# mathaiml5/NBody-simulation-parallel

Measured on AMD Instinct MI355X. Metric: body-pair interactions/sec at N=2^20 (all-pairs force + kick/drift step), higher is better.
Workload: dtype f32

## Files before the change

### include/nbody_hip.h

```cpp
#ifndef NBODY_HIP_H
#define NBODY_HIP_H

#include <stddef.h>
#include <stdint.h>

#ifdef __cplusplus
extern "C" {
#endif
#if defined(__GNUC__)
#pragma GCC visibility push(default)
#endif

#define NBX_ABI_VERSION 5

enum {
    NBX_OK = 0,
    NBX_ERR_INVALID = 1,
    NBX_ERR_NO_DEVICE = 2,
    NBX_ERR_HIP = 3,
    NBX_ERR_ALLOC = 4,
    NBX_ERR_STATE = 5
};

#define NBX_REFERENCE_G 4.471e-21
// ... 123 lines not shown
int nbx_ctx_get_accel(nbx_ctx* ctx, float* accel_out);
int nbx_ctx_download_bodies(nbx_ctx* ctx, void* bodies, size_t body_stride_bytes);

int nbx_ctx_energy(nbx_ctx* ctx, double G, double* kinetic, double* potential);

int nbx_ctx_synchronize(nbx_ctx* ctx);

int nbx_ctx_set_tuning(nbx_ctx* ctx, int source_splits, int variant);
enum { NBX_CLOSE_CANDIDATE_PAIRS = 0, NBX_CLOSE_SORTED_CELLS = 1, NBX_CLOSE_GUARDED_KERNEL = 2, NBX_CLOSE_NONE = 3 };
int nbx_ctx_close_set_mode(nbx_ctx* ctx, int* mode, unsigned* candidates_seen, unsigned* bad_seen);

int nbx_ctx_set_softening(nbx_ctx* ctx, double epsilon);
enum { NBX_FORCE_LAW_REFERENCE = 0, NBX_FORCE_LAW_NEWTON = 1 };
int nbx_ctx_set_law(nbx_ctx* ctx, int law);
int nbx_ctx_set_refine(nbx_ctx* ctx, double rel_tolerance, double sigma_factor);
int nbx_ctx_refine_stats(nbx_ctx* ctx, unsigned* selected, unsigned* refined);
int nbx_ctx_get_aux(nbx_ctx* ctx, double* out);
int nbx_ctx_effective_tuning(nbx_ctx* ctx, int* variant, int* source_splits);
int nbx_num_variants(void);
const char* nbx_variant_name(int variant);
int nbx_default_variant(void);

int nbx_ctx_kernel_time(nbx_ctx* ctx, float* mean_ms, int* launches);
int nbx_ctx_refine_time(nbx_ctx* ctx, float* total_ms);

int nbx_variant_kernel_symbol(int variant, int dim, int mixed_mode, char* buf, size_t len);
int nbx_ctx_enable_clock_stamps(nbx_ctx* ctx, int on);
int nbx_ctx_shader_clock(nbx_ctx* ctx, double* median_mhz, double* min_mhz, double* max_mhz, int* workgroups);
int nbx_measure_valu_ceiling(int device, double target_ms, double* tflops, double* shader_mhz);

// ... 31 lines not shown
```

### nbody-simulation-parallel_amd/capi.py

```python
from __future__ import annotations

import ctypes
import os
from typing import Optional, Tuple

import numpy as np

NBX_OK = 0
NBX_ERR_INVALID, NBX_ERR_NO_DEVICE, NBX_ERR_HIP, NBX_ERR_ALLOC, NBX_ERR_STATE = 1, 2, 3, 4, 5
SRC_ALL, SRC_LOCAL, SRC_REMOTE = 0, 1, 2
REFERENCE_G = 4.471e-21

_PKG_DIR = os.path.dirname(os.path.abspath(__file__))
LIB_PATH = os.environ.get("NBODY_HIP_LIBRARY") or os.path.join(_PKG_DIR, "libnbody_hip.so")

_c = ctypes
_vp, _sz, _i, _d = _c.c_void_p, _c.c_size_t, _c.c_int, _c.c_double
_pf, _pd, _pi = _c.POINTER(_c.c_float), _c.POINTER(_c.c_double), _c.POINTER(_c.c_int)
ABI = [
    ("nbx_abi_version", _i, []),
    ("nbx_strerror", _c.c_char_p, [_i]),
    ("nbx_last_error_detail", _c.c_char_p, []),
    ("nbx_device_count", _i, [_pi]),
    ("nbx_warmup", _i, [_i]),
# ... 49 lines not shown
    ("nbx_ctx_compute_accel", _i, [_vp, _i]),
    ("nbx_ctx_kick_drift", _i, [_vp, _d, _d]),
    ("nbx_ctx_kick_drift2", _i, [_vp, _d, _d, _d]),
    ("nbx_ctx_step_kdk", _i, [_vp, _d, _d, _i]),
    ("nbx_ctx_step", _i, [_vp, _d, _d, _i]),
    ("nbx_ctx_get_forces", _i, [_vp, _d, _vp]),
    ("nbx_ctx_accuracy", _i, [_vp, _d, _vp, _pd]),
    ("nbx_ctx_get_accel", _i, [_vp, _vp]),
    ("nbx_ctx_download_bodies", _i, [_vp, _vp, _sz]),
    ("nbx_ctx_energy", _i, [_vp, _d, _pd, _pd]),
    ("nbx_ctx_synchronize", _i, [_vp]),
    ("nbx_ctx_set_tuning", _i, [_vp, _i, _i]),
    ("nbx_ctx_set_softening", _i, [_vp, _d]),
    ("nbx_ctx_set_law", _i, [_vp, _i]),
    ("nbx_ctx_set_refine", _i, [_vp, _d, _d]),
    ("nbx_ctx_refine_stats", _i, [_vp, _c.POINTER(_c.c_uint), _c.POINTER(_c.c_uint)]),
    ("nbx_ctx_get_aux", _i, [_vp, _vp]),
    ("nbx_ctx_close_set_mode", _i, [_vp, _pi, _c.POINTER(_c.c_uint), _c.POINTER(_c.c_uint)]),
    ("nbx_ctx_effective_tuning", _i, [_vp, _pi, _pi]),
    ("nbx_num_variants", _i, []),
    ("nbx_variant_name", _c.c_char_p, [_i]),
    ("nbx_default_variant", _i, []),
    ("nbx_ctx_kernel_time", _i, [_vp, _pf, _pi]),
    ("nbx_ctx_refine_time", _i, [_vp, _pf]),
    ("nbx_variant_kernel_symbol", _i, [_i, _i, _i, _c.c_char_p, _sz]),
    ("nbx_ctx_enable_clock_stamps", _i, [_vp, _i]),
    ("nbx_ctx_shader_clock", _i, [_vp, _pd, _pd, _pd, _pi]),
    ("nbx_measure_valu_ceiling", _i, [_i, _d, _pd, _pd]),
    ("nbx_node_create", _i, [_c.POINTER(_vp), _i, _pi, _i, _sz, _i]),
    ("nbx_node_destroy", _i, [_vp]),
# ... 438 lines not shown

    def set_softening(self, epsilon: float):
        self._ck(self.lib.nbx_ctx_set_softening(self.h, float(epsilon)), "nbx_ctx_set_softening")

    def close_set_mode(self) -> Tuple[str, int, int]:
        m, a, b = ctypes.c_int(0), ctypes.c_uint(0), ctypes.c_uint(0)
        self._ck(self.lib.nbx_ctx_close_set_mode(self.h, ctypes.byref(m), ctypes.byref(a), ctypes.byref(b)), "nbx_ctx_close_set_mode")
        return ("candidate_pairs", "sorted_cells", "guarded_kernel", "none")[m.value], a.value, b.value

    def set_law(self, law: int):
        self._ck(self.lib.nbx_ctx_set_law(self.h, int(law)), "nbx_ctx_set_law")

    def set_refine(self, rel_tolerance: float, sigma_factor: float = 0.0):
        self._ck(self.lib.nbx_ctx_set_refine(self.h, float(rel_tolerance), float(sigma_factor)), "nbx_ctx_set_refine")

    def refine_stats(self) -> Tuple[int, int]:
        a, b = ctypes.c_uint(0), ctypes.c_uint(0)
        self._ck(self.lib.nbx_ctx_refine_stats(self.h, ctypes.byref(a), ctypes.byref(b)), "nbx_ctx_refine_stats")
        return a.value, b.value

    def aux(self) -> np.ndarray:
        out = np.empty(self.count, dtype=np.float64)
        self._ck(self.lib.nbx_ctx_get_aux(self.h, out.ctypes.data), "nbx_ctx_get_aux")
        return out

    def effective_tuning(self) -> Tuple[str, int]:
        v, s = ctypes.c_int(0), ctypes.c_int(0)
        self._ck(self.lib.nbx_ctx_effective_tuning(self.h, ctypes.byref(v), ctypes.byref(s)), "nbx_ctx_effective_tuning")
        return self.lib.nbx_variant_name(v.value).decode(), s.value

# ... 185 lines not shown
```

### nbody-simulation-parallel_amd/csrc/force_kernel.hip

```cpp
#include "nbx_internal.h"

#include <climits>
#include <cmath>

namespace nbx {
namespace {


typedef float f2 __attribute__((ext_vector_type(2)));

template <int D>
__device__ __forceinline__ void interact(float sx, float sy, float sz, float sm,
                                         float ix, float iy, float iz,
                                         float& ax, float& ay, float& az) {
    const float dx = sx - ix;
    const float dy = sy - iy;
    float r2 = dx * dx;
    r2 = __builtin_fmaf(dy, dy, r2);
    float dz = 0.0f;
    if (D == 3) {
        dz = sz - iz;
        r2 = __builtin_fmaf(dz, dz, r2);
    }
    const float r2g = (r2 < kR2SkipF) ? __builtin_inff() : r2;
// ... 709 lines not shown
                for (int s = 1; s < a.splits; ++s) a.acc[((size_t)s * D + k) * a.pad + i] = 0.0f;
            }
        }
    }
}

template <int D>
__global__ __launch_bounds__(256) void refine_select_kernel(KArgs a) {
    const unsigned gid = blockIdx.x * 256u + threadIdx.x;
    const unsigned i = gid >> 2, part = gid & 3u;
    const bool in = i < a.count;
    double t = 0.0;
    if (in && part < (unsigned)D) {
#pragma unroll 8
        for (int s = 0; s < a.splits; ++s) t += (double)a.acc[((size_t)s * D + part) * a.pad + i];
        t = t * t;
    } else if (in && part == 3u) {
#pragma unroll 8
        for (int s = 0; s < a.grid_slices; ++s) t += (double)a.qsum[(size_t)s * a.pad + i];
    }
    const int base = (int)(threadIdx.x & 63u) & ~3;
    const double n2 = __shfl(t, base) + __shfl(t, base + 1) + (D == 3 ? __shfl(t, base + 2) : 0.0);
    const double Q = __shfl(t, base + 3);
    if (in && part == 0u) {
        const bool suspect = a.bad_flag[i] != 0u || !(Q * a.refine_c2 <= n2);
        if (suspect) {
            const unsigned slot = atomicAdd(&a.counters[3], 1u);
            if (slot < a.strict_cap) a.strict_list[slot] = i;
        }
    }
// ... 1 lines not shown

template <int D>
__global__ __launch_bounds__(256) void refine_fold_kernel(KArgs a) {
    const StrictLayout sl = strict_layout<D>(a);
    const unsigned lane = threadIdx.x & 63u;
    const unsigned long long items = (unsigned long long)sl.n * (unsigned)D;
    for (unsigned long long item = blockIdx.x * 4u + (threadIdx.x >> 6); item < items; item += gridDim.x * 4u) {
        const unsigned slot = (unsigned)(item / (unsigned)D), k = (unsigned)(item - (unsigned long long)slot * (unsigned)D);
        double v = 0.0;
        for (unsigned y = lane; y < sl.slices; y += 64u) v += a.strict_acc[((size_t)y * D + k) * sl.stride + slot];
        for (int off = 32; off > 0; off >>= 1) v += __shfl_xor(v, off);
        const unsigned i = a.strict_list[slot];
        const float hi = (float)v;
        if (lane == 0u) {
            a.acc[(size_t)k * a.pad + i] = hi;
            if (a.splits > 1) a.acc[((size_t)D + k) * a.pad + i] = (float)(v - (double)hi);
        }
        for (unsigned sp = 2u + lane; sp < (unsigned)a.splits; sp += 64u) a.acc[((size_t)sp * D + k) * a.pad + i] = 0.0f;
    }
}

template <int D, int SOFT>
__global__ __launch_bounds__(256, 8) void potential_kernel(KArgs a) {
    constexpr int TPL = 2;
    __shared__ float4 tile[2][kTile];
    const unsigned tid = threadIdx.x;
    unsigned bx, by;
    xcd_tile(bx, by);
    const unsigned tgt0 = bx * (256u * TPL) + tid;
    const float* __restrict__ tp = a.pos_all + (size_t)a.tgt_chunk * D * a.pad;
    float ix[TPL], iy[TPL], iz[TPL];
// ... 113 lines not shown
```

### nbody-simulation-parallel_amd/csrc/force_launch.hip

```cpp
#include "nbx_internal.h"
#include "sym_plan.h"

#include <cxxabi.h>

#include <climits>
#include <cstdio>
#include <cstdlib>
#include <cstring>
#include <vector>

namespace nbx {
namespace {

struct Table {
    std::vector<KernelVariant> v;
    int def = 0, def_exact = 0, def_two_rcp = 0;
    CloseKernels ck;
    Table() {
        int n = 0;
        const KernelVariant* a = kernel_variants(&n);
        for (int i = 0; i < n; ++i) v.push_back(a[i]);
        v.push_back(sym_kernel_variant());
        v.push_back(sym_dpp_kernel_variant());
        for (size_t i = 0; i < v.size(); ++i) {
// ... 74 lines not shown
    a.pad = L.pad;
    a.count = L.count;
    a.tiles_per_chunk = L.pad / kTile;
    a.total_tiles = (unsigned)L.vchunks * a.tiles_per_chunk;
    if (L.splits % V.planes != 0) return hipErrorInvalidValue;
    const unsigned slices = (unsigned)(L.splits / V.planes);
    a.tiles_per_split = (a.total_tiles + slices - 1) / slices;
    a.tgt_chunk = L.tgt_chunk;
    a.chunk_first = L.chunk_first;
    a.chunk_skip = L.chunk_skip;
    a.accumulate = L.accumulate;
    a.splits = L.splits;
    a.grid_slices = (int)slices;
    a.qsum = L.qsum;
    a.strict_list = nullptr; a.strict_acc = nullptr; a.strict_cap = 0; a.strict_slices = 0; a.strict_budget = 0; a.refine_c2 = 0.0;
    a.clk = nullptr;
    a.cand_list = L.cand_list;
    a.cand_pos = L.cand_pos;
    a.bad_list = L.bad_list;
    a.bad_flag = L.bad_flag;
    a.counters = L.counters;
    a.close_acc = L.close_acc;
    a.src_cand_pos = L.src_cand_pos;
    a.src_stride = (unsigned)L.n_chunks * L.pad;
    a.n_total = (unsigned)L.n_total;
    a.shard_len = (unsigned)L.shard_len;
    a.eps2 = L.eps2;
    a.clk = V.stamps ? L.clk : nullptr;
    const bool soft = L.eps2 > 0.0f;
    if (soft && !(V.fast && V.soft2 && V.soft3)) return hipErrorInvalidValue;
// ... 76 lines not shown
    const AccelLaunch& L = R.base;
    if ((dim != 2 && dim != 3) || L.pad == 0 || L.pad % kPadQuantum != 0 || L.splits < 1 || L.n_chunks < 1 || L.count > L.pad ||
        !L.acc || !L.qsum || !L.counters || !L.bad_flag || R.grid_slices < 1 || L.splits % R.grid_slices != 0)
        return hipErrorInvalidValue;
    a = KArgs{};
    a.pos_all = L.pos_all; a.mass_all = L.mass_all; a.acc = L.acc; a.pad = L.pad; a.count = L.count;
    a.tiles_per_chunk = L.pad / kTile;
    a.total_tiles = (unsigned)L.n_chunks * a.tiles_per_chunk;
    a.tgt_chunk = L.tgt_chunk; a.chunk_first = 0; a.chunk_skip = INT_MAX; a.accumulate = 0;
    a.splits = L.splits;
    a.grid_slices = R.grid_slices;
    a.bad_flag = L.bad_flag; a.counters = L.counters; a.qsum = L.qsum;
    a.strict_list = R.strict_list; a.strict_acc = R.strict_acc; a.strict_cap = R.strict_cap; a.strict_slices = R.strict_slices;
    a.strict_budget = R.strict_budget;
    a.refine_c2 = R.c2;
    return hipSuccess;
}
}

hipError_t launch_refine(int dim, const RefineLaunch& R, hipStream_t stream) {
    KArgs a;
    hipError_t e = refine_args(dim, R, a);
    if (e != hipSuccess) return e;
    if (!R.strict_list || !R.strict_acc || R.strict_cap < R.base.pad || R.strict_slices < 1 || R.strict_slices > 256 ||
        (unsigned)R.strict_slices > a.total_tiles || R.strict_budget < (unsigned long long)dim * R.base.pad)
        return hipErrorInvalidValue;
    a.tiles_per_split = 0;
    if ((e = hipMemsetAsync(a.counters + 3, 0, sizeof(unsigned), stream)) != hipSuccess) return e;
    if (a.count == 0) return hipSuccess;
    const int di = dim - 2;
// ... 34 lines not shown
```

### nbody-simulation-parallel_amd/csrc/force_sym_kernel.hip

```cpp
#include "nbx_internal.h"
#include "sym_plan.h"

namespace nbx {
namespace {

typedef float f2 __attribute__((ext_vector_type(2)));

__device__ __forceinline__ float ror1(float v) {
    const int i = __builtin_bit_cast(int, v);
    return __builtin_bit_cast(float, __builtin_amdgcn_update_dpp(i, i, 0x13C, 0xF, 0xF, false));
}
__device__ __forceinline__ void ror1(f2& v) { v.x = ror1(v.x); v.y = ror1(v.y); }

enum { kRotDpp = 0, kRotLds = 1 };
template <int D> struct SymLanes { static constexpr int kVisitors = (D == 3) ? 2 : 1; };
constexpr int kSymBlockSteps = 8;
template <int D> struct RotBuf {
    static constexpr unsigned kEntries = 72u;
    static constexpr unsigned kPlanes = (unsigned)SymLanes<D>::kVisitors;
    static constexpr unsigned kWaveBytes = kPlanes * kEntries * (unsigned)sizeof(float4);
};

template <int D, int PAIRS>
__device__ __forceinline__ void sym_step(const f2 vxy, const f2 vzm, const f2 (&ix)[PAIRS], const f2 (&iy)[PAIRS],
// ... 119 lines not shown
    __shared__ __attribute__((aligned(16))) char smem[kSumBytes + kVisBytes + kRotBytes];
    double2* __restrict__ sums = reinterpret_cast<double2*>(smem);
    float4* __restrict__ vbuf = reinterpret_cast<float4*>(smem + kSumBytes);

    SymPlan P;
    if (!sym_make_plan(a.pad, &P) || P.B != gridDim.x || P.S != gridDim.y) return;
    if (VPL == 2 && P.G < 2u) return;
    const unsigned A = blockIdx.x, s = blockIdx.y;
    const unsigned tid = threadIdx.x, lane = tid & 63u, wave = tid >> 6;
    unsigned long long clk_r0 = 0, clk_t0 = 0;
    if (a.clk) {
        clk_r0 = __builtin_amdgcn_s_memrealtime();
        clk_t0 = __builtin_amdgcn_s_memtime();
        __builtin_amdgcn_s_waitcnt(0xC07F);
    }
    const size_t pad = a.pad;
    const float* __restrict__ tp = a.pos_all + (size_t)a.tgt_chunk * D * pad;
    const float* __restrict__ mp = a.mass_all + (size_t)a.tgt_chunk * pad;
    const f2 bias = f2{kTiny, kTiny};
    const size_t slot_stride = 2 * (size_t)D * pad;

    const unsigned delta = ((unsigned)__builtin_amdgcn_update_dpp((int)lane, (int)lane, 0x13C, 0xF, 0xF, false) - lane) & 63u;
    const unsigned rpos = ((0u - delta) * lane) & 63u;
    const unsigned vrot = kSumBytes + kVisBytes + ((ROT == kRotLds) ? wave * RotBuf<D>::kWaveBytes : 0u);

    if (sym_clears_last_slot(P, A)) {
        float* __restrict__ hi = a.acc + (size_t)(P.S + P.K - 1u) * slot_stride;
        const unsigned len = kSymSuper / P.S;
        for (unsigned t = tid; t < len; t += 256u) {
            const size_t v = (size_t)A * kSymSuper + (size_t)s * len + t;
            if (v < pad) {
#pragma unroll
                for (int k = 0; k < 2 * D; ++k) hi[(size_t)k * pad + v] = 0.0f;
                if (QS) a.qsum[(size_t)(P.S + P.K - 1u) * pad + v] = 0.0f;
            }
        }
    }

    for (unsigned hp = 0; hp < kSymSuper / kSymHomePass; ++hp) {
        const unsigned h0 = A * kSymSuper + hp * kSymHomePass;
        if (h0 >= a.pad) break;
        const unsigned tgt0 = h0 + tid;
        f2 ix[PAIRS], iy[PAIRS], iz[PAIRS], hm[PAIRS], qq[QS ? PAIRS : 1];
#pragma unroll
        for (int q = 0; q < PAIRS; ++q) {
            const unsigned i0 = tgt0 + (2 * q) * 256u, i1 = i0 + 256u;
            ix[q] = f2{tp[i0], tp[i1]};
            iy[q] = f2{tp[pad + i0], tp[pad + i1]};
            iz[q] = (D == 3) ? f2{tp[2 * pad + i0], tp[2 * pad + i1]} : f2{0.f, 0.f};
            hm[q] = f2{mp[i0], mp[i1]};
            if (QS) qq[q] = f2{0.f, 0.f};
        }
#pragma unroll
        for (int c = 0; c < PAIRS * D; ++c) sums[c * 256 + tid] = double2{0.0, 0.0};

        SymWalk nw;
        nw.k = 0u; nw.c = ~0u;
        bool more = sym_next_chunk(P, A, s, &nw);
        f2 nxy = f2{0.f, 0.f}, nzm = f2{0.f, 0.f};
        f2 nvx = f2{0.f, 0.f}, nvy = f2{0.f, 0.f}, nvz = f2{0.f, 0.f}, nvm = f2{0.f, 0.f};
        if (more) {
            if constexpr (VPL == 2) load_visitor_pair(tp, mp, a.pad, nw.first + lane, nvx, nvy, nvz, nvm);
            else load_visitor<D>(tp, mp, a.pad, nw.first + lane, nxy, nzm);
        }
        while (more) {
            const SymWalk cw = nw;
            f2 ox[PAIRS], oy[PAIRS], oz[PAIRS];
#pragma unroll
            for (int q = 0; q < PAIRS; ++q) ox[q] = oy[q] = oz[q] = f2{0.f, 0.f};
            if constexpr (VPL == 2) {
#pragma unroll 1
                for (unsigned g = 0; g < cw.groups; g += 2u) {
// ... 158 lines not shown
            }
#pragma unroll
            for (int q = 0; q < PAIRS; ++q) {
                double2 v = sums[(q * D + 0) * 256 + tid];
                v.x += (double)ox[q].x; v.y += (double)ox[q].y;
                sums[(q * D + 0) * 256 + tid] = v;
                v = sums[(q * D + 1) * 256 + tid];
                v.x += (double)oy[q].x; v.y += (double)oy[q].y;
                sums[(q * D + 1) * 256 + tid] = v;
                if (D == 3) {
                    v = sums[(q * D + 2) * 256 + tid];
                    v.x += (double)oz[q].x; v.y += (double)oz[q].y;
                    sums[(q * D + 2) * 256 + tid] = v;
                }
            }
            if (!cw.two_sided) continue;
            __syncthreads();
            if (tid < cw.groups * kSymGroup) {
                const unsigned g = tid >> 6;
                const size_t v = (size_t)cw.first + tid;
                const float4 b0 = vbuf[(0u * kSymChunkGroups + g) * kSymGroup + lane], b1 = vbuf[(1u * kSymChunkGroups + g) * kSymGroup + lane];
                const float4 b2 = vbuf[(2u * kSymChunkGroups + g) * kSymGroup + lane], b3 = vbuf[(3u * kSymChunkGroups + g) * kSymGroup + lane];
                float* __restrict__ hi = a.acc + (size_t)(P.S + cw.k - 1u) * slot_stride;
                float* __restrict__ lo = hi + (size_t)D * pad;
                double rx = -((((double)b0.x + (double)b1.x) + (double)b2.x) + (double)b3.x);
                double ry = -((((double)b0.y + (double)b1.y) + (double)b2.y) + (double)b3.y);
                double rz = -((((double)b0.z + (double)b1.z) + (double)b2.z) + (double)b3.z);
                if (hp != 0u) {
                    rx += (double)hi[v] + (double)lo[v];
                    ry += (double)hi[pad + v] + (double)lo[pad + v];
                    if (D == 3) rz += (double)hi[2 * pad + v] + (double)lo[2 * pad + v];
                }
                store_hi_lo(hi, lo, v, rx);
                store_hi_lo(hi, lo, pad + v, ry);
                if (D == 3) store_hi_lo(hi, lo, 2 * pad + v, rz);
                if (QS) {
                    float* __restrict__ qo = a.qsum + (size_t)(P.S + cw.k - 1u) * pad + v;
                    const float qv = ((b0.w + b1.w) + b2.w) + b3.w;
                    *qo = (hp != 0u) ? *qo + qv : qv;
                }
            }
            __syncthreads();
        }

        float* __restrict__ hi = a.acc + (size_t)s * slot_stride;
        float* __restrict__ lo = hi + (size_t)D * pad;
        float* __restrict__ qout = QS ? a.qsum + (size_t)s * pad : nullptr;
#pragma unroll
        for (int q = 0; q < PAIRS; ++q) {
            const double2 vx = sums[(q * D + 0) * 256 + tid], vy = sums[(q * D + 1) * 256 + tid];
            const double2 vz = (D == 3) ? sums[(q * D + (D == 3 ? 2 : 0)) * 256 + tid] : double2{0.0, 0.0};
#pragma unroll
            for (int h = 0; h < 2; ++h) {
                const unsigned i = tgt0 + (2 * q + h) * 256u;
                if (!a.bad_flag[i]) {
                    store_hi_lo(hi, lo, i, h ? vx.y : vx.x);
                    store_hi_lo(hi, lo, pad + i, h ? vy.y : vy.x);
                    if (D == 3) store_hi_lo(hi, lo, 2 * pad + i, h ? vz.y : vz.x);
                    if (QS) qout[i] = h ? qq[q].y : qq[q].x;
                } else if (QS) {
                    qout[i] = __builtin_inff();
                }
            }
        }
    }
    if (a.clk) {
        const unsigned long long t1 = __builtin_amdgcn_s_memtime(), r1 = __builtin_amdgcn_s_memrealtime();
        if (tid == 0) {
            const size_t wg = (size_t)blockIdx.y * gridDim.x + blockIdx.x;
// ... 28 lines not shown
```

### nbody-simulation-parallel_amd/csrc/nbx_api.hip

```cpp
#include "../../include/nbody_hip.h"
#include "nbx_internal.h"
#include "nbx_ctx.h"
#include "device_block.h"

#include <algorithm>
#include <atomic>
#include <climits>
#include <cstdio>
#include <cstdlib>
#include <cstring>
#include <mutex>
#include <new>
#include <string>
#include <utility>
#include <vector>

using namespace nbx;

namespace {

thread_local std::string g_detail;
}

namespace nbx {
// ... 296 lines not shown
            c->close_splits_alloc = c->splits;
        }
    }
    if (refine_active(c, c->variant) || variant_writes_aux(c->variant)) {
        if (!(c->qsum && c->qsum_slices_alloc >= c->splits)) {
            if ((rc = dev_release(c, c->qsum, (size_t)c->qsum_slices_alloc * c->pad * sizeof(float)))) return rc;
            if ((rc = dev_alloc(c, &c->qsum, (size_t)c->splits * c->pad * sizeof(float)))) return rc;
            c->qsum_slices_alloc = c->splits;
        }
        if (refine_active(c, c->variant) && !c->strict_list) {
            size_t list_bytes = 0, acc_bytes = 0;
            strict_sizes(c, &list_bytes, &acc_bytes);
            if ((rc = dev_alloc(c, &c->strict_list, list_bytes))) return rc;
            if ((rc = dev_alloc(c, &c->strict_acc, acc_bytes))) return rc;
        }
    }
    return NBX_OK;
}

RefineLaunch refine_launch(const nbx_ctx* c) {
    RefineLaunch R = {};
    R.base.pos_all = c->pos_all; R.base.mass_all = c->mass_all; R.base.acc = c->acc; R.base.pad = c->pad;
    R.base.count = (unsigned)c->count; R.base.tgt_chunk = c->shard; R.base.splits = c->splits; R.base.n_chunks = c->n_shards;
    R.base.counters = c->counters; R.base.bad_flag = c->bad_flag; R.base.qsum = c->qsum;
    R.strict_list = c->strict_list; R.strict_acc = c->strict_acc; R.strict_cap = c->strict_cap; R.strict_slices = c->strict_slices;
    R.strict_budget = c->strict_budget;
    const bool three_level = variant_planes(c->variant) == 2;
    const double sigma = c->refine_sigma > 0.0 ? c->refine_sigma
                         : three_level ? (c->dim == 2 ? kRefineSigmaDefault2D : kRefineSigmaDefault3D)
                                       : (c->dim == 2 ? kRefineSigmaTwoLevel2D : kRefineSigmaTwoLevel3D);
    const double r = sigma * kUnitRoundoffF32 / c->refine_tol;
    R.c2 = r * r;
    R.grid_slices = c->splits / variant_planes(c->variant);
    return R;
}

constexpr int kPollEverySteps = 16;

int poll_close_counters(nbx_ctx* c, int steps) {
    if (c->capturing || c->softening > 0.0 || c->force_exact || !c->counters || !variant_is_fast(c->variant)) return NBX_OK;
    if (c->counters_pending && hipEventQuery(c->counters_ev) == hipSuccess) {
// ... 217 lines not shown
    CTX_TRY(take_stream(device, &c->own_stream));
    c->stream = c->own_stream;
    {
        const size_t body = (size_t)(2 * dim + 1) * sizeof(double);
        const int launched = effective_variant(c);
        const int splits = variant_is_sym(launched) ? variant_sym_slots(launched, c->pad) : auto_splits(c, c->variant);
        size_t want = 2 * arena_round((size_t)dim * pad * sizeof(double)) + arena_round(pad * sizeof(double));
        want += arena_round(n_total * body + 16) + arena_round(3 * sizeof(unsigned long long));
        want += 2 * arena_round((size_t)splits * variant_planes(c->variant) * dim * pad * sizeof(float));
        want += 3 * arena_round(pad * sizeof(unsigned)) + arena_round((size_t)dim * pad * sizeof(float)) + arena_round(16)
                + arena_round((size_t)dim * n_shards * pad * sizeof(float));
        if (n_shards == 1) want += arena_round((size_t)dim * pad * sizeof(float)) + arena_round(pad * sizeof(float));
        if (c->refine_tol > 0.0) {
            size_t list_bytes = 0, acc_bytes = 0;
            strict_sizes(c, &list_bytes, &acc_bytes);
            want += arena_round((size_t)splits * variant_planes(c->variant) * pad * sizeof(float)) + arena_round(list_bytes) + arena_round(acc_bytes);
        }
        if (want <= ((size_t)64 << 30)) {
            CTX_TRY((hipError_t)nbx_block::ctx_pool().take(device, want, &c->arena, &c->arena_bytes));
        }
    }
#define CTX_ALLOC(ptr, bytes) do { int r_ = dev_alloc(c, &(ptr), (bytes)); if (r_) { nbx_ctx_destroy(c); return r_; } } while (0)
    CTX_ALLOC(c->x64, (size_t)dim * pad * sizeof(double));
    CTX_ALLOC(c->v64, (size_t)dim * pad * sizeof(double));
    CTX_ALLOC(c->m64, pad * sizeof(double));
    CTX_ALLOC(c->facts, 3 * sizeof(unsigned long long));
#undef CTX_ALLOC
    c->ev0.assign(kEventPairs, nullptr);
    c->ev1.assign(kEventPairs, nullptr);
    c->ev2.assign(kEventPairs, nullptr);
    c->ev2_set.assign(kEventPairs, 0);
// ... 139 lines not shown
    if (!c) return fail(NBX_ERR_INVALID, "ctx is null");
    if (law != NBX_FORCE_LAW_REFERENCE && law != NBX_FORCE_LAW_NEWTON) return fail(NBX_ERR_INVALID, "unknown force law");
    c->law = law;
    c->have_accel = false;
    c->tgt_cand_valid = 0; c->bad_list_pass = -1;
    return NBX_OK;
}

int nbx_ctx_set_refine(nbx_ctx* c, double rel_tolerance, double sigma_factor) {
    if (!c) return fail(NBX_ERR_INVALID, "ctx is null");
    const char* why = "";
    if (!refine_args_ok(rel_tolerance, sigma_factor, &why)) return fail(NBX_ERR_INVALID, why);
    c->refine_tol = rel_tolerance;
    c->refine_sigma = sigma_factor;
    c->have_accel = false;
    return NBX_OK;
}

int nbx_ctx_refine_stats(nbx_ctx* c, unsigned* selected, unsigned* refined) {
    if (!c) return fail(NBX_ERR_INVALID, "ctx is null");
    if (!c->have_accel || !refine_active(c, c->variant) || !c->qsum) return fail(NBX_ERR_STATE, "no mixed-mode evaluation on the device (nbx_ctx_set_refine, then compute)");
    if (!c->refined) return fail(NBX_ERR_STATE, "the accelerations on the device are a LOCAL pass only");
    int rc = set_device(c);
    if (rc) return rc;
    unsigned n = 0;
    HIP_TRY(hipMemcpyAsync(&n, c->counters + 3, sizeof n, hipMemcpyDeviceToHost, c->stream));
    HIP_TRY(hipStreamSynchronize(c->stream));
    if (selected) *selected = n;
    if (refined) *refined = n;
    return NBX_OK;
// ... 120 lines not shown
        }
        c->bulk_steps_done += c->ev_used;
        c->ev_used = 0;
    }
    const bool timed = !c->capturing;
    if (timed && !c->ev0[c->ev_used]) {
        HIP_TRY(hipEventCreate(&c->ev0[c->ev_used]));
        HIP_TRY(hipEventCreate(&c->ev1[c->ev_used]));
    }
    const bool refine_now = refine && (which != NBX_SRC_LOCAL || c->n_shards == 1);
    if (timed) { L.ev_start = c->ev0[c->ev_used]; L.ev_stop = c->ev1[c->ev_used]; c->ev2_set[c->ev_used] = 0; }
    HIP_TRY(launch_accel(c->dim, L, c->stream));
    ++c->launches_since_query;
    c->have_accel = true;
    c->refined = false;
    if (refine_now) {
        HIP_TRY(launch_refine(c->dim, refine_launch(c), c->stream));
        if (timed) {
            if (!c->ev2[c->ev_used]) HIP_TRY(hipEventCreate(&c->ev2[c->ev_used]));
            HIP_TRY(hipEventRecord(c->ev2[c->ev_used], c->stream));
            c->ev2_set[c->ev_used] = 1;
        }
        c->refined = true;
    }
    if (timed) ++c->ev_used;
    return NBX_OK;
}

int nbx_ctx_kick_drift2(nbx_ctx* c, double G, double dt_kick, double dt_drift) {
    if (!c) return fail(NBX_ERR_INVALID, "ctx is null");
    if (!c->have_accel) return fail(NBX_ERR_STATE, "compute accelerations before kick_drift");
    int rc = set_device(c);
    if (rc) return rc;
    KickDriftArgs k;
    k.acc = c->acc; k.splits = c->splits; k.dim = c->dim; k.pad = c->pad; k.count = c->count; k.G = c->law ? -G : G;
    k.dt_kick = dt_kick; k.dt_drift = dt_drift;
    k.x64 = c->x64; k.v64 = c->v64; k.m64 = c->m64;
    k.pos_chunk = c->pos_all + (size_t)c->shard * c->dim * c->pad;
    if (dt_drift != 0.0) {
        rc = poll_close_counters(c, 1);
        if (rc) return rc;
    }
    HIP_TRY(launch_kick_drift(k, c->stream));
    if (dt_drift != 0.0) {
        c->have_accel = false;
        c->tgt_cand_valid = 0; c->bad_list_pass = -1;
    }
    return NBX_OK;
}

int nbx_ctx_kick_drift(nbx_ctx* c, double G, double dt) { return nbx_ctx_kick_drift2(c, G, dt, dt); }

static bool capture_step(nbx_ctx* c, double G, double dt) {
    if (c->step_exec && c->graph_G == G && c->graph_dt == dt && c->graph_variant == c->variant &&
        c->graph_splits == c->splits && c->graph_stream == c->stream && c->graph_eps == c->softening && c->graph_law == c->law && c->graph_hash == c->hash_refine &&
        c->graph_refine_tol == c->refine_tol && c->graph_refine_sigma == c->refine_sigma && c->graph_clk == (c->clk_on ? c->clk : nullptr))
        return true;
    if (c->step_exec) { (void)hipGraphExecDestroy(c->step_exec); c->step_exec = nullptr; }
    if (hipStreamBeginCapture(c->stream, hipStreamCaptureModeThreadLocal) != hipSuccess) { (void)hipGetLastError(); return false; }
    c->capturing = true;
    c->tgt_cand_valid = 0; c->bad_list_pass = -1;
    int rc = nbx_ctx_compute_accel(c, NBX_SRC_ALL);
    if (!rc) rc = nbx_ctx_kick_drift(c, G, dt);
    c->capturing = false;
    hipGraph_t graph = nullptr;
    const hipError_t e = hipStreamEndCapture(c->stream, &graph);
    if (rc || e != hipSuccess || !graph) { if (graph) (void)hipGraphDestroy(graph); (void)hipGetLastError(); return false; }
    const hipError_t ei = hipGraphInstantiate(&c->step_exec, graph, nullptr, nullptr, 0);
    (void)hipGraphDestroy(graph);
    if (ei != hipSuccess) { c->step_exec = nullptr; (void)hipGetLastError(); return false; }
    c->graph_eps = c->softening; c->graph_law = c->law; c->graph_hash = c->hash_refine;
    c->graph_refine_tol = c->refine_tol; c->graph_refine_sigma = c->refine_sigma;
    c->graph_clk = c->clk_on ? c->clk : nullptr;
    c->graph_G = G; c->graph_dt = dt; c->graph_variant = c->variant; c->graph_splits = c->splits; c->graph_stream = c->stream;
    return true;
}

int nbx_ctx_step(nbx_ctx* c, double G, double dt, int nsteps) {
    if (!c) return fail(NBX_ERR_INVALID, "ctx is null");
    if (c->n_shards != 1) return fail(NBX_ERR_STATE, "nbx_ctx_step drives single-shard contexts only");
    if (nsteps < 0) return fail(NBX_ERR_INVALID, "nsteps < 0");
    if (!c->uploaded) return fail(NBX_ERR_STATE, "upload bodies before stepping");
    int s = 0;
    if (nsteps >= kGraphMinSteps && !c->no_graphs) {
        int rc = set_device(c);
        if (rc) return rc;
// ... 250 lines not shown
```

### nbody-simulation-parallel_amd/csrc/nbx_ctx.h

```cpp
#ifndef NBX_CTX_H
#define NBX_CTX_H

#include <vector>

#include "nbx_internal.h"

struct nbx_ctx {
    unsigned long long id = 0;
    int device = 0, dim = 3, n_shards = 1, shard = 0;
    size_t n_total = 0, shard_len = 0, count = 0;
    unsigned pad = 0;
    int splits = 1, variant = 0;
    bool splits_user = false;
    int user_slices = 0;
    bool uploaded = false, have_accel = false;
    bool shard_staged = false;
    unsigned long long pending_facts[3] = {0, 0, 0};
    hipStream_t own_stream = nullptr, stream = nullptr;
    float* pos_all = nullptr;
    float* mass_all = nullptr;
    bool own_gather = true;
    double *x64 = nullptr, *v64 = nullptr, *m64 = nullptr;
    unsigned long long* facts = nullptr;
    float* acc = nullptr;
// ... 12 lines not shown
    unsigned* counters_host = nullptr;
    hipEvent_t counters_ev = nullptr;
    bool counters_pending = false;
    int steps_since_poll = 0;
    unsigned last_cand = 0, last_bad = 0;
    double refine_tol = 0.0;
    double refine_sigma = 0.0;
    float* qsum = nullptr;
    int qsum_slices_alloc = 0;
    unsigned* strict_list = nullptr;
    double* strict_acc = nullptr;
    unsigned strict_cap = 0;
    int strict_slices = 0;
    unsigned long long strict_budget = 0;
    bool refined = false;
    float* phi = nullptr;
    hipGraphExec_t step_exec = nullptr;
    double graph_G = 0.0, graph_dt = 0.0, graph_eps = 0.0, graph_refine_tol = 0.0, graph_refine_sigma = 0.0;
    int graph_law = 0;
    bool graph_hash = false;
    int graph_variant = -1, graph_splits = 0;
    hipStream_t graph_stream = nullptr;
    bool capturing = false;
    hipEvent_t bulk0 = nullptr, bulk1 = nullptr;
    int bulk_steps = 0;
    double bulk_ms_done = 0.0;
    int bulk_steps_done = 0;
    bool no_graphs = false;
    int tgt_cand_valid = 0;
    int bad_list_pass = -1;
    int law = 0;
    double softening = 0.0;
    double mass_max = 0.0;
    bool extent_ok = false;
    bool force_exact = false;
// ... 41 lines not shown
```

### nbody-simulation-parallel_amd/csrc/nbx_internal.h

```cpp
#ifndef NBX_INTERNAL_H
#define NBX_INTERNAL_H

#include <hip/hip_runtime.h>
#include <stddef.h>
#include <stdint.h>

namespace nbx {

constexpr int kTile = 256;
constexpr int kPadQuantum = 4096;

constexpr float kR2SkipF = 1.0e-10f;
static_assert((double)kR2SkipF >= 1e-10, "fp32 threshold must not round below the fp64 one");
constexpr double kR2Skip64 = 1.0e-10;

constexpr float kTiny = 0x1p-47f;
constexpr float kCloseCoord = 16384.0f;
constexpr float kBadR2 = 1.0e-6f;
constexpr unsigned kRefineLimit = 131072;
constexpr unsigned long long kRefinePairLimit = 1ull << 36;
constexpr double kFastMaxMass = 1.0e10;
constexpr double kOneRcpMaxCoord = 1.0e8;
constexpr int kCloseBlocksX = 32;

// ... 63 lines not shown
    unsigned* __restrict__ bad_list;
    unsigned* __restrict__ bad_flag;
    unsigned* __restrict__ counters;
    float* __restrict__ close_acc;
    float* __restrict__ src_cand_pos;
    unsigned src_stride;
    unsigned n_total, shard_len;
    float eps2;
    float* __restrict__ qsum;
    unsigned* __restrict__ strict_list;
    double* __restrict__ strict_acc;
    unsigned strict_cap;
    int strict_slices;
    unsigned long long strict_budget;
    double refine_c2;
    unsigned long long* __restrict__ clk;
};

struct KernelVariant {
    const char* name;
    int tpl;
    void (*k2)(KArgs);
    void (*k3)(KArgs);
    int fast;
    int max_tiles_per_slice;
    int needs_extent;
    void (*soft2)(KArgs);
    void (*soft3)(KArgs);
    void (*newton2)(KArgs);
    void (*newton3)(KArgs);
// ... 13 lines not shown
CloseKernels close_kernels();

size_t hash_temp_bytes(unsigned capacity);
hipError_t hash_refine(int dim, const KArgs& a, const HashWork& h, hipStream_t stream);

hipError_t launch_accel(int dim, const AccelLaunch& a, hipStream_t stream);
struct RefineLaunch {
    AccelLaunch base;
    unsigned* strict_list;
    double* strict_acc;
    unsigned strict_cap;
    int strict_slices;
    unsigned long long strict_budget;
    double c2;
    int grid_slices;
};
hipError_t launch_refine(int dim, const RefineLaunch& R, hipStream_t stream);
hipError_t launch_potential(int dim, const AccelLaunch& a, hipStream_t stream);
int num_variants();
const char* variant_name(int variant);
int variant_tpl(int variant);
int variant_is_fast(int variant);
int variant_max_tiles_per_slice(int variant);
int variant_needs_extent(int variant);
int variant_has_law_builds(int variant);
int variant_planes(int variant);
int variant_has_qsum(int variant);
int variant_writes_aux(int variant);
int variant_is_sym(int variant);
int variant_sym_slots(int variant, unsigned pad);
// ... 19 lines not shown
    double* m64;
    int only_own;
    size_t n_own;
    unsigned long long* facts;
};
hipError_t launch_pack(const PackArgs& p, hipStream_t stream);

struct KickDriftArgs {
    const float* acc;
    int splits, dim;
    unsigned pad;
    size_t count;
    double G, dt_kick, dt_drift;
    double* x64; double* v64; const double* m64;
    float* pos_chunk;
};
hipError_t launch_kick_drift(const KickDriftArgs& k, hipStream_t stream);
struct SlotKickArgs {
    const double* sums;
    const uint32_t* body_slot;
    uint32_t pslots;
    int dim;
    unsigned pad;
    bool drift;
    size_t count;
    double signedG, dt_kick, dt_drift;
    double* x64; double* v64; const double* m64;
    float* pos_chunk;
};
static_assert(offsetof(SlotKickArgs, drift) == 28 && offsetof(SlotKickArgs, count) == 32 && sizeof(SlotKickArgs) == 96,
// ... 38 lines not shown
```

### nbody-simulation-parallel_amd/csrc/state_kernels.hip

```cpp
#include "nbx_internal.h"

namespace nbx {
namespace {

__device__ __forceinline__ double sum_partials(const float* __restrict__ acc, int splits, int dim,
                                               unsigned pad, int k, size_t l) {
    double a = 0.0;
#pragma unroll 8
    for (int s = 0; s < splits; ++s) a += (double)acc[((size_t)s * dim + k) * pad + l];
    return a;
}

__global__ __launch_bounds__(256) void pack_kernel(PackArgs p) {
    __shared__ unsigned long long s_mass, s_coord;
    __shared__ unsigned s_close;
    if (threadIdx.x == 0) { s_mass = 0ull; s_coord = 0ull; s_close = 0u; }
    __syncthreads();
    const size_t b = (size_t)blockIdx.x * 256 + threadIdx.x;
    if (b < (p.only_own ? (size_t)p.pad : (size_t)p.n_shards * p.pad)) {
        const int g = p.only_own ? p.shard : (int)(b / p.pad);
        const size_t l = p.only_own ? b : b - (size_t)g * p.pad;
        const size_t id = p.only_own ? l : (size_t)g * p.shard_len + l;
        const bool real = p.only_own ? (l < p.n_own) : ((l < p.shard_len) && (id < p.n_total));
        const double* __restrict__ src = p.raw + id * p.stride_d;
// ... 28 lines not shown
    }
    __syncthreads();
    if (threadIdx.x == 0) {
        if (s_mass > *(volatile unsigned long long*)&p.facts[0]) atomicMax(&p.facts[0], s_mass);
        if (s_coord > *(volatile unsigned long long*)&p.facts[1]) atomicMax(&p.facts[1], s_coord);
        if (s_close) atomicAdd(&p.facts[2], (unsigned long long)s_close);
    }
}

__global__ __launch_bounds__(256) void kick_drift_kernel(KickDriftArgs a) {
    const size_t l = (size_t)blockIdx.x * 256 + threadIdx.x;
    if (l >= a.count) return;
    const int k = (int)blockIdx.y;
    const double m = a.m64[l];
    const double gm = a.G * m;
    const double acc = sum_partials(a.acc, a.splits, a.dim, a.pad, k, l);
    const double F = -(gm * acc);
    double v = a.v64[(size_t)k * a.pad + l];
    double x = a.x64[(size_t)k * a.pad + l];
    v += (F / m) * a.dt_kick;
    x += v * a.dt_drift;
    a.v64[(size_t)k * a.pad + l] = v;
    a.x64[(size_t)k * a.pad + l] = x;
    a.pos_chunk[(size_t)k * a.pad + l] = (float)x;
}

template <bool DRIFT>
__global__ __launch_bounds__(256) void kick_drift_slots_kernel(SlotKickArgs a) {
    const size_t l = (size_t)blockIdx.x * 256 + threadIdx.x;
    if (l >= a.count) return;
    const int k = (int)blockIdx.y;
// ... 327 lines not shown
```

### nbody-simulation-parallel_amd/csrc/sym_plan.h

```cpp
#ifndef NBX_SYM_PLAN_H
#define NBX_SYM_PLAN_H

#if defined(__HIPCC__) || defined(__CUDACC__)
#define NBX_SYM_HD __host__ __device__
#else
#define NBX_SYM_HD
#endif

namespace nbx {

constexpr unsigned kSymSuper = 8192;
constexpr unsigned kSymHomePass = 2048;
constexpr unsigned kSymGroup = 64;
constexpr unsigned kSymChunkGroups = 4;
constexpr unsigned kSymMaxSlots = 128;
constexpr unsigned kSymWantGroups = 4096;

struct SymPlan {
    unsigned pad;
    unsigned B;
    unsigned S;
    unsigned K;
    unsigned G;
};
// ... 33 lines not shown
    const unsigned gc = p.G < kSymChunkGroups ? p.G : kSymChunkGroups;
    const unsigned chunks = p.G / gc;
    unsigned k = w->k, c = w->c + 1u;
    for (; k <= p.K; ++k, c = 0u) {
        unsigned block; bool two;
        if (!sym_visit(p, A, k, &block, &two)) continue;
        const unsigned first = block * kSymSuper + s * (kSymSuper / p.S) + c * gc * kSymGroup;
        if (c >= chunks || first >= p.pad) continue;
        w->k = k; w->c = c; w->first = first; w->groups = gc; w->two_sided = two;
        return true;
    }
    w->k = k; w->c = 0u;
    return false;
}

}
#endif
```

Before: 6297 billion.

## Exploit symmetry within home superblock and reuse refined double sums in kick

The symmetric force kernel now rotates the home-pass order per source slice and classifies each within-superblock meeting as one-sided, two-sided or skipped. Pairs inside the home superblock are then computed once and the reaction is written back, instead of being evaluated from both sides. Separately, the refine pass stores the combined double-precision accelerations into a new sum64 buffer, and kick/drift reads it rather than re-summing split partials. The changes add an extra allocation, more complex ownership logic with possible correctness risk, and extra global writes in refine.

Result: no change. 6340 billion, median of 6 (+0.7%).

```diff
diff --git a/include/nbody_hip.h b/include/nbody_hip.h
--- a/include/nbody_hip.h
+++ b/include/nbody_hip.h
@@ -161,6 +161,7 @@
 enum { NBX_FORCE_LAW_REFERENCE = 0, NBX_FORCE_LAW_NEWTON = 1 };
 int nbx_ctx_set_law(nbx_ctx* ctx, int law);
 int nbx_ctx_set_refine(nbx_ctx* ctx, double rel_tolerance, double sigma_factor);
+int nbx_ctx_set_sum_once(nbx_ctx* ctx, int on);
 int nbx_ctx_refine_stats(nbx_ctx* ctx, unsigned* selected, unsigned* refined);
 int nbx_ctx_get_aux(nbx_ctx* ctx, double* out);
 int nbx_ctx_effective_tuning(nbx_ctx* ctx, int* variant, int* source_splits);
diff --git a/nbody-simulation-parallel_amd/capi.py b/nbody-simulation-parallel_amd/capi.py
--- a/nbody-simulation-parallel_amd/capi.py
+++ b/nbody-simulation-parallel_amd/capi.py
@@ -87,6 +87,7 @@
     ("nbx_ctx_set_softening", _i, [_vp, _d]),
     ("nbx_ctx_set_law", _i, [_vp, _i]),
     ("nbx_ctx_set_refine", _i, [_vp, _d, _d]),
+    ("nbx_ctx_set_sum_once", _i, [_vp, _i]),
     ("nbx_ctx_refine_stats", _i, [_vp, _c.POINTER(_c.c_uint), _c.POINTER(_c.c_uint)]),
     ("nbx_ctx_get_aux", _i, [_vp, _vp]),
     ("nbx_ctx_close_set_mode", _i, [_vp, _pi, _c.POINTER(_c.c_uint), _c.POINTER(_c.c_uint)]),
@@ -555,6 +556,9 @@
     def set_refine(self, rel_tolerance: float, sigma_factor: float = 0.0):
         self._ck(self.lib.nbx_ctx_set_refine(self.h, float(rel_tolerance), float(sigma_factor)), "nbx_ctx_set_refine")
 
+    def set_sum_once(self, on: bool = True):
+        self._ck(self.lib.nbx_ctx_set_sum_once(self.h, 1 if on else 0), "nbx_ctx_set_sum_once")
+
     def refine_stats(self) -> Tuple[int, int]:
         a, b = ctypes.c_uint(0), ctypes.c_uint(0)
         self._ck(self.lib.nbx_ctx_refine_stats(self.h, ctypes.byref(a), ctypes.byref(b)), "nbx_ctx_refine_stats")
diff --git a/nbody-simulation-parallel_amd/csrc/force_kernel.hip b/nbody-simulation-parallel_amd/csrc/force_kernel.hip
--- a/nbody-simulation-parallel_amd/csrc/force_kernel.hip
+++ b/nbody-simulation-parallel_amd/csrc/force_kernel.hip
@@ -747,6 +747,7 @@
     if (in && part < (unsigned)D) {
 #pragma unroll 8
         for (int s = 0; s < a.splits; ++s) t += (double)a.acc[((size_t)s * D + part) * a.pad + i];
+        if (a.sum64) a.sum64[(size_t)part * a.pad + i] = t;
         t = t * t;
     } else if (in && part == 3u) {
 #pragma unroll 8
@@ -778,7 +779,9 @@
         const float hi = (float)v;
         if (lane == 0u) {
             a.acc[(size_t)k * a.pad + i] = hi;
-            if (a.splits > 1) a.acc[((size_t)D + k) * a.pad + i] = (float)(v - (double)hi);
+            const float lo = (float)(v - (double)hi);
+            if (a.splits > 1) a.acc[((size_t)D + k) * a.pad + i] = lo;
+            if (a.sum64) a.sum64[(size_t)k * a.pad + i] = (a.splits > 1) ? (0.0 + (double)hi) + (double)lo : 0.0 + (double)hi;
         }
         for (unsigned sp = 2u + lane; sp < (unsigned)a.splits; sp += 64u) a.acc[((size_t)sp * D + k) * a.pad + i] = 0.0f;
     }
diff --git a/nbody-simulation-parallel_amd/csrc/force_launch.hip b/nbody-simulation-parallel_amd/csrc/force_launch.hip
--- a/nbody-simulation-parallel_amd/csrc/force_launch.hip
+++ b/nbody-simulation-parallel_amd/csrc/force_launch.hip
@@ -112,6 +112,7 @@
     a.grid_slices = (int)slices;
     a.qsum = L.qsum;
     a.strict_list = nullptr; a.strict_acc = nullptr; a.strict_cap = 0; a.strict_slices = 0; a.strict_budget = 0; a.refine_c2 = 0.0;
+    a.sum64 = nullptr;
     a.clk = nullptr;
     a.cand_list = L.cand_list;
     a.cand_pos = L.cand_pos;
@@ -218,6 +219,7 @@
     a.strict_list = R.strict_list; a.strict_acc = R.strict_acc; a.strict_cap = R.strict_cap; a.strict_slices = R.strict_slices;
     a.strict_budget = R.strict_budget;
     a.refine_c2 = R.c2;
+    a.sum64 = R.sum64;
     return hipSuccess;
 }
 }
diff --git a/nbody-simulation-parallel_amd/csrc/force_sym_kernel.hip b/nbody-simulation-parallel_amd/csrc/force_sym_kernel.hip
--- a/nbody-simulation-parallel_amd/csrc/force_sym_kernel.hip
+++ b/nbody-simulation-parallel_amd/csrc/force_sym_kernel.hip
@@ -157,6 +157,7 @@
         clk_t0 = __builtin_amdgcn_s_memtime();
         __builtin_amdgcn_s_waitcnt(0xC07F);
     }
+    asm volatile("" : "+v"(clk_r0), "+v"(clk_t0));
     const size_t pad = a.pad;
     const float* __restrict__ tp = a.pos_all + (size_t)a.tgt_chunk * D * pad;
     const float* __restrict__ mp = a.mass_all + (size_t)a.tgt_chunk * pad;
@@ -180,9 +181,11 @@
         }
     }
 
-    for (unsigned hp = 0; hp < kSymSuper / kSymHomePass; ++hp) {
+    const unsigned hp_first = sym_first_home_pass(P, A, s);
+    for (unsigned pi = 0; pi < kSymSuper / kSymHomePass; ++pi) {
+        const unsigned hp = (hp_first + pi) % (kSymSuper / kSymHomePass);
         const unsigned h0 = A * kSymSuper + hp * kSymHomePass;
-        if (h0 >= a.pad) break;
+        if (h0 >= a.pad) continue;
         const unsigned tgt0 = h0 + tid;
         f2 ix[PAIRS], iy[PAIRS], iz[PAIRS], hm[PAIRS], qq[QS ? PAIRS : 1];
 #pragma unroll
@@ -198,7 +201,8 @@
         for (int c = 0; c < PAIRS * D; ++c) sums[c * 256 + tid] = double2{0.0, 0.0};
 
         SymWalk nw;
-        nw.k = 0u; nw.c = ~0u;
+        unsigned own_v = (unsigned)sym_walk_start(P, A, s, hp, &nw);
+        asm volatile("" : "+v"(own_v));
         bool more = sym_next_chunk(P, A, s, &nw);
         f2 nxy = f2{0.f, 0.f}, nzm = f2{0.f, 0.f};
         f2 nvx = f2{0.f, 0.f}, nvy = f2{0.f, 0.f}, nvz = f2{0.f, 0.f}, nvm = f2{0.f, 0.f};
@@ -387,19 +391,21 @@
                     sums[(q * D + 2) * 256 + tid] = v;
                 }
             }
-            if (!cw.two_sided) continue;
+            if (!(cw.two_sided || __builtin_amdgcn_readfirstlane(own_v) == (unsigned)kSymOwnTwoSided)) continue;
+            const unsigned vslot_id = cw.k != 0u ? P.S + cw.k - 1u : s;
+            const bool onto = cw.k != 0u ? pi != 0u : true;
             __syncthreads();
             if (tid < cw.groups * kSymGroup) {
                 const unsigned g = tid >> 6;
                 const size_t v = (size_t)cw.first + tid;
                 const float4 b0 = vbuf[(0u * kSymChunkGroups + g) * kSymGroup + lane], b1 = vbuf[(1u * kSymChunkGroups + g) * kSymGroup + lane];
                 const float4 b2 = vbuf[(2u * kSymChunkGroups + g) * kSymGroup + lane], b3 = vbuf[(3u * kSymChunkGroups + g) * kSymGroup + lane];
-                float* __restrict__ hi = a.acc + (size_t)(P.S + cw.k - 1u) * slot_stride;
+                float* __restrict__ hi = a.acc + (size_t)vslot_id * slot_stride;
                 float* __restrict__ lo = hi + (size_t)D * pad;
                 double rx = -((((double)b0.x + (double)b1.x) + (double)b2.x) + (double)b3.x);
                 double ry = -((((double)b0.y + (double)b1.y) + (double)b2.y) + (double)b3.y);
                 double rz = -((((double)b0.z + (double)b1.z) + (double)b2.z) + (double)b3.z);
-                if (hp != 0u) {
+                if (onto) {
                     rx += (double)hi[v] + (double)lo[v];
                     ry += (double)hi[pad + v] + (double)lo[pad + v];
                     if (D == 3) rz += (double)hi[2 * pad + v] + (double)lo[2 * pad + v];
@@ -408,9 +414,9 @@
                 store_hi_lo(hi, lo, pad + v, ry);
                 if (D == 3) store_hi_lo(hi, lo, 2 * pad + v, rz);
                 if (QS) {
-                    float* __restrict__ qo = a.qsum + (size_t)(P.S + cw.k - 1u) * pad + v;
+                    float* __restrict__ qo = a.qsum + (size_t)vslot_id * pad + v;
                     const float qv = ((b0.w + b1.w) + b2.w) + b3.w;
-                    *qo = (hp != 0u) ? *qo + qv : qv;
+                    *qo = onto ? *qo + qv : qv;
                 }
             }
             __syncthreads();
@@ -419,13 +425,15 @@
         float* __restrict__ hi = a.acc + (size_t)s * slot_stride;
         float* __restrict__ lo = hi + (size_t)D * pad;
         float* __restrict__ qout = QS ? a.qsum + (size_t)s * pad : nullptr;
+        unsigned row0 = tgt0;
+        asm volatile("" : "+v"(row0));
 #pragma unroll
         for (int q = 0; q < PAIRS; ++q) {
             const double2 vx = sums[(q * D + 0) * 256 + tid], vy = sums[(q * D + 1) * 256 + tid];
             const double2 vz = (D == 3) ? sums[(q * D + (D == 3 ? 2 : 0)) * 256 + tid] : double2{0.0, 0.0};
 #pragma unroll
             for (int h = 0; h < 2; ++h) {
-                const unsigned i = tgt0 + (2 * q + h) * 256u;
+                const unsigned i = row0 + (2 * q + h) * 256u;
                 if (!a.bad_flag[i]) {
                     store_hi_lo(hi, lo, i, h ? vx.y : vx.x);
                     store_hi_lo(hi, lo, pad + i, h ? vy.y : vy.x);
diff --git a/nbody-simulation-parallel_amd/csrc/nbx_api.hip b/nbody-simulation-parallel_amd/csrc/nbx_api.hip
--- a/nbody-simulation-parallel_amd/csrc/nbx_api.hip
+++ b/nbody-simulation-parallel_amd/csrc/nbx_api.hip
@@ -334,6 +334,10 @@
             if ((rc = dev_alloc(c, &c->strict_list, list_bytes))) return rc;
             if ((rc = dev_alloc(c, &c->strict_acc, acc_bytes))) return rc;
         }
+        if (refine_active(c, c->variant) && !c->sum64) {
+            if ((rc = dev_alloc(c, &c->sum64, (size_t)c->dim * c->pad * sizeof(double)))) return rc;
+            c->sum64_current = false;
+        }
     }
     return NBX_OK;
 }
@@ -345,6 +349,7 @@
     R.base.counters = c->counters; R.base.bad_flag = c->bad_flag; R.base.qsum = c->qsum;
     R.strict_list = c->strict_list; R.strict_acc = c->strict_acc; R.strict_cap = c->strict_cap; R.strict_slices = c->strict_slices;
     R.strict_budget = c->strict_budget;
+    R.sum64 = c->sum_once ? c->sum64 : nullptr;
     const bool three_level = variant_planes(c->variant) == 2;
     const double sigma = c->refine_sigma > 0.0 ? c->refine_sigma
                          : three_level ? (c->dim == 2 ? kRefineSigmaDefault2D : kRefineSigmaDefault3D)
@@ -592,7 +597,8 @@
         if (c->refine_tol > 0.0) {
             size_t list_bytes = 0, acc_bytes = 0;
             strict_sizes(c, &list_bytes, &acc_bytes);
-            want += arena_round((size_t)splits * variant_planes(c->variant) * pad * sizeof(float)) + arena_round(list_bytes) + arena_round(acc_bytes);
+            want += arena_round((size_t)splits * variant_planes(c->variant) * pad * sizeof(float)) + arena_round(list_bytes) + arena_round(acc_bytes)
+                    + arena_round((size_t)dim * pad * sizeof(double));
         }
         if (want <= ((size_t)64 << 30)) {
             CTX_TRY((hipError_t)nbx_block::ctx_pool().take(device, want, &c->arena, &c->arena_bytes));
@@ -762,6 +768,12 @@
     c->refine_tol = rel_tolerance;
     c->refine_sigma = sigma_factor;
     c->have_accel = false;
+    return NBX_OK;
+}
+
+int nbx_ctx_set_sum_once(nbx_ctx* c, int on) {
+    if (!c) return fail(NBX_ERR_INVALID, "ctx is null");
+    c->sum_once = on != 0;
     return NBX_OK;
 }
 
@@ -912,8 +924,11 @@
     ++c->launches_since_query;
     c->have_accel = true;
     c->refined = false;
+    c->sum64_current = false;
     if (refine_now) {
-        HIP_TRY(launch_refine(c->dim, refine_launch(c), c->stream));
+        const RefineLaunch R = refine_launch(c);
+        HIP_TRY(launch_refine(c->dim, R, c->stream));
+        c->sum64_current = R.sum64 != nullptr && c->count != 0;
         if (timed) {
             if (!c->ev2[c->ev_used]) HIP_TRY(hipEventCreate(&c->ev2[c->ev_used]));
             HIP_TRY(hipEventRecord(c->ev2[c->ev_used], c->stream));
@@ -935,6 +950,7 @@
     k.dt_kick = dt_kick; k.dt_drift = dt_drift;
     k.x64 = c->x64; k.v64 = c->v64; k.m64 = c->m64;
     k.pos_chunk = c->pos_all + (size_t)c->shard * c->dim * c->pad;
+    if (c->sum_once && c->sum64_current) k.sum64 = c->sum64;
     if (dt_drift != 0.0) {
         rc = poll_close_counters(c, 1);
         if (rc) return rc;
@@ -951,7 +967,7 @@
 
 static bool capture_step(nbx_ctx* c, double G, double dt) {
     if (c->step_exec && c->graph_G == G && c->graph_dt == dt && c->graph_variant == c->variant &&
-        c->graph_splits == c->splits && c->graph_stream == c->stream && c->graph_eps == c->softening && c->graph_law == c->law && c->graph_hash == c->hash_refine &&
+        c->graph_splits == c->splits && c->graph_stream == c->stream && c->graph_eps == c->softening && c->graph_law == c->law && c->graph_hash == c->hash_refine && c->graph_sum_once == c->sum_once &&
         c->graph_refine_tol == c->refine_tol && c->graph_refine_sigma == c->refine_sigma && c->graph_clk == (c->clk_on ? c->clk : nullptr))
         return true;
     if (c->step_exec) { (void)hipGraphExecDestroy(c->step_exec); c->step_exec = nullptr; }
@@ -967,7 +983,7 @@
     const hipError_t ei = hipGraphInstantiate(&c->step_exec, graph, nullptr, nullptr, 0);
     (void)hipGraphDestroy(graph);
     if (ei != hipSuccess) { c->step_exec = nullptr; (void)hipGetLastError(); return false; }
-    c->graph_eps = c->softening; c->graph_law = c->law; c->graph_hash = c->hash_refine;
+    c->graph_eps = c->softening; c->graph_law = c->law; c->graph_hash = c->hash_refine; c->graph_sum_once = c->sum_once;
     c->graph_refine_tol = c->refine_tol; c->graph_refine_sigma = c->refine_sigma;
     c->graph_clk = c->clk_on ? c->clk : nullptr;
     c->graph_G = G; c->graph_dt = dt; c->graph_variant = c->variant; c->graph_splits = c->splits; c->graph_stream = c->stream;
diff --git a/nbody-simulation-parallel_amd/csrc/nbx_ctx.h b/nbody-simulation-parallel_amd/csrc/nbx_ctx.h
--- a/nbody-simulation-parallel_amd/csrc/nbx_ctx.h
+++ b/nbody-simulation-parallel_amd/csrc/nbx_ctx.h
@@ -50,11 +50,14 @@
     int strict_slices = 0;
     unsigned long long strict_budget = 0;
     bool refined = false;
+    double* sum64 = nullptr;
+    bool sum_once = true;
+    bool sum64_current = false;
     float* phi = nullptr;
     hipGraphExec_t step_exec = nullptr;
     double graph_G = 0.0, graph_dt = 0.0, graph_eps = 0.0, graph_refine_tol = 0.0, graph_refine_sigma = 0.0;
     int graph_law = 0;
-    bool graph_hash = false;
+    bool graph_hash = false, graph_sum_once = true;
     int graph_variant = -1, graph_splits = 0;
     hipStream_t graph_stream = nullptr;
     bool capturing = false;
diff --git a/nbody-simulation-parallel_amd/csrc/nbx_internal.h b/nbody-simulation-parallel_amd/csrc/nbx_internal.h
--- a/nbody-simulation-parallel_amd/csrc/nbx_internal.h
+++ b/nbody-simulation-parallel_amd/csrc/nbx_internal.h
@@ -101,6 +101,7 @@
     int strict_slices;
     unsigned long long strict_budget;
     double refine_c2;
+    double* __restrict__ sum64;
     unsigned long long* __restrict__ clk;
 };
 
@@ -144,6 +145,7 @@
     unsigned long long strict_budget;
     double c2;
     int grid_slices;
+    double* sum64 = nullptr;
 };
 hipError_t launch_refine(int dim, const RefineLaunch& R, hipStream_t stream);
 hipError_t launch_potential(int dim, const AccelLaunch& a, hipStream_t stream);
@@ -193,6 +195,7 @@
     double G, dt_kick, dt_drift;
     double* x64; double* v64; const double* m64;
     float* pos_chunk;
+    const double* sum64 = nullptr;
 };
 hipError_t launch_kick_drift(const KickDriftArgs& k, hipStream_t stream);
 struct SlotKickArgs {
diff --git a/nbody-simulation-parallel_amd/csrc/state_kernels.hip b/nbody-simulation-parallel_amd/csrc/state_kernels.hip
--- a/nbody-simulation-parallel_amd/csrc/state_kernels.hip
+++ b/nbody-simulation-parallel_amd/csrc/state_kernels.hip
@@ -66,7 +66,7 @@
     const int k = (int)blockIdx.y;
     const double m = a.m64[l];
     const double gm = a.G * m;
-    const double acc = sum_partials(a.acc, a.splits, a.dim, a.pad, k, l);
+    const double acc = a.sum64 ? a.sum64[(size_t)k * a.pad + l] : sum_partials(a.acc, a.splits, a.dim, a.pad, k, l);
     const double F = -(gm * acc);
     double v = a.v64[(size_t)k * a.pad + l];
     double x = a.x64[(size_t)k * a.pad + l];
diff --git a/nbody-simulation-parallel_amd/csrc/sym_plan.h b/nbody-simulation-parallel_amd/csrc/sym_plan.h
--- a/nbody-simulation-parallel_amd/csrc/sym_plan.h
+++ b/nbody-simulation-parallel_amd/csrc/sym_plan.h
@@ -71,5 +71,44 @@
     return false;
 }
 
+enum SymOwn { kSymOwnOneSided = 0, kSymOwnTwoSided = 1, kSymOwnSkip = 2 };
+
+NBX_SYM_HD inline unsigned sym_home_passes(const SymPlan& p, unsigned A) {
+    const unsigned left = p.pad - A * kSymSuper;
+    return (left < kSymSuper ? left : kSymSuper) / kSymHomePass;
+}
+
+NBX_SYM_HD inline bool sym_own_by_pass(const SymPlan& p) { return kSymSuper / p.S <= kSymHomePass; }
+
+NBX_SYM_HD inline SymOwn sym_own_meeting(const SymPlan& p, unsigned A, unsigned hp, unsigned first) {
+    if (!sym_own_by_pass(p)) return kSymOwnOneSided;
+    const unsigned n = sym_home_passes(p, A);
+    const unsigned hs = (first - A * kSymSuper) / kSymHomePass;
+    if (hp == hs) return kSymOwnOneSided;
+    if (n == 2u) return hp == 0u ? kSymOwnTwoSided : kSymOwnSkip;
+    if ((hp + 1u) % n == hs) return kSymOwnTwoSided;
+    if ((hp + 2u) % n == hs) {
+        const unsigned lo = hp < hs ? hp : hs;
+        const unsigned owner = (lo & 1u) == 0u ? lo : lo + 2u;
+        return hp == owner ? kSymOwnTwoSided : kSymOwnSkip;
+    }
+    return kSymOwnSkip;
+}
+
+NBX_SYM_HD inline unsigned sym_first_home_pass(const SymPlan& p, unsigned A, unsigned s) {
+    if (!sym_own_by_pass(p)) return 0u;
+    const unsigned off = s * (kSymSuper / p.S);
+    if (A * kSymSuper + off >= p.pad) return 0u;
+    return off / kSymHomePass;
+}
+
+NBX_SYM_HD inline SymOwn sym_walk_start(const SymPlan& p, unsigned A, unsigned s, unsigned hp, SymWalk* w) {
+    const unsigned first = A * kSymSuper + s * (kSymSuper / p.S);
+    const SymOwn own = first < p.pad ? sym_own_meeting(p, A, hp, first) : kSymOwnSkip;
+    w->k = own == kSymOwnSkip ? 1u : 0u;
+    w->c = ~0u;
+    return own;
+}
+
 }
 #endif
```
